# gjgjh/PTZ-Calib

Measured on AMD Instinct MI355X. Metric: LM iterations/sec (PTZ-IBA global BA, 200-view synthetic PTZ rig), higher is better.
Workload: dtype f64

## Files before the change

### __graft_entry__.py

```python
from __future__ import annotations

import importlib.util
import os
import subprocess
import sys

ROOT = os.path.dirname(os.path.abspath(__file__))
PKG_DIR = os.path.join(ROOT, "ptz-calib_amd")


def load_package():
    if "ptz_calib_amd" in sys.modules:
        return sys.modules["ptz_calib_amd"]
    spec = importlib.util.spec_from_file_location("ptz_calib_amd", os.path.join(PKG_DIR, "__init__.py"),
                                                  submodule_search_locations=[PKG_DIR])
    mod = importlib.util.module_from_spec(spec)
    sys.modules["ptz_calib_amd"] = mod
    spec.loader.exec_module(mod)
    return mod


def load_oracle():
    odir = os.path.join(ROOT, "oracle")
    if odir not in sys.path:
        sys.path.insert(0, odir)
    import oracle_py
    return oracle_py


def build() -> None:
    env = dict(os.environ)
    subprocess.check_call(["make", "-C", os.path.join(PKG_DIR, "csrc"), "-j4"], env=env)
    host = os.path.join(PKG_DIR, "host")
    if os.path.exists(os.path.join(host, "Makefile")):
        subprocess.check_call(["make", "-C", host], env=env)
    subprocess.check_call(["make", "-C", os.path.join(ROOT, "oracle")], env=env)
    harness = os.path.join(ROOT, "tests", "cpu_harness")
    for name in ("factor_harness", "homography_harness", "krt_cov_harness", "ba_cov_harness", "ba_cov_georef_harness", "pass_shape_harness",
                 "xcd_map_harness", "ba_trim_harness", "krt_trim_harness", "desc_match_harness", "desc_guided_harness", "reloc_assemble_harness",
                 "desc_shortlist_harness"):
        subprocess.check_call(["g++", "-O2", "-ffp-contract=off", "-shared", "-fPIC", "-o",
                               os.path.join(harness, "lib%s.so" % name), os.path.join(harness, name + ".cc")])
    pkg = load_package()
    pkg.api.lib()
    for name in pkg.api.EXPORTS:
        getattr(pkg.api.lib(), name)


def smoke() -> None:
    import numpy as np
    import torch

    assert torch.cuda.is_available(), "smoke() needs cuda:0"
    pkg = load_package()
    orc = load_oracle()
# ... 68 lines not shown
```

### include/ptz_calib_amd.h

```cpp
#ifndef PTZ_CALIB_AMD_H
#define PTZ_CALIB_AMD_H

#include <stdint.h>

#ifdef __cplusplus
extern "C" {
#endif

#define PTZ_CAM_DIM 15

#define PTZ_OK 0
#define PTZ_EINVAL (-1)
#define PTZ_ENODEVICE (-2)
#define PTZ_ENOMEM (-3)
#define PTZ_EUNSUPPORTED (-4)
#define PTZ_ELIMIT (-5)
#define PTZ_ENOOBS (-6)

#define PTZ_BA_PTZRay 0
#define PTZ_BA_PTZRayDist 1
#define PTZ_BA_PTZRayFxfyDist 2
#define PTZ_BA_PTZRayDistDisp 3
#define PTZ_KRT_F 0
#define PTZ_KRT_FDist 1
// ... 93 lines not shown
                       int32_t device_id, ptz_rig** out);
void ptz_rig_destroy(ptz_rig* rig);
typedef struct ptz_rig_view {
  const ptz_rig* rig;
  int32_t n_cam;
  const int32_t* cam_image;
} ptz_rig_view;
int32_t ptz_ba_batch_create_views(int32_t n, const ptz_rig_view* views, int32_t factor_type, const ptz_lm_options* opt,
                                  ptz_ba_batch** out);
int32_t ptz_ba_batch_set_state_pix2ray(ptz_ba_batch* b, const double* cam, const double* rkinv);
int32_t ptz_debug_batch_structure_hash(ptz_ba_batch* b, uint64_t* hash);
int32_t ptz_debug_batch_initial_rays(ptz_ba_batch* b, double* ray);

int32_t ptz_chol_solve_batch(int32_t count, int32_t n, const double* A, const double* rhs, double* x, int32_t* fail,
                             int32_t device_id, double* device_ms);

int32_t ptz_mfma_f64_peak(int32_t device_id, double* tflops);
int32_t ptz_ba_plan_tile_order(int32_t nt, int32_t first_dense, const uint8_t* mask, int32_t* perm, int32_t* lanes,
                               int32_t* sched, int32_t* n_steps);

int32_t ptz_hbm_bandwidth(int32_t device_id, double* read_gbps, double* copy_gbps);

int32_t ptz_krt_solve_batch(int32_t n_query, const int64_t* match_ptr, const float* uv_ref, const float* uv_cur,
                            const double* cam_ref, double* cam_cur, int32_t factor_type, double max_reproj_error,
                            const ptz_lm_options* opt, ptz_lm_summary* summaries, int32_t* accepted,
                            double* device_ms);

int32_t ptz_krt_solve_batch_2d3d(int32_t n_query, const int64_t* match_ptr, const float* uv_ref, const float* uv_cur,
                                 const int64_t* point_ptr, const float* pts2d, const double* pts3d, const double* cam_ref,
                                 double* cam_cur, int32_t factor_type, double max_reproj_error, const ptz_lm_options* opt,
// ... 282 lines not shown
```

### ptz-calib_amd/api.py

```python
from __future__ import annotations

import ctypes as C
import os

import numpy as np

_HERE = os.path.dirname(os.path.abspath(__file__))
LIB_PATH = os.environ.get("PTZCALIB_LIB", os.path.join(_HERE, "libptzcalib_hip.so"))

CONVERGENCE, NO_CONVERGENCE, FAILURE = 0, 1, 2
BA_PTZRay, BA_PTZRayDist, BA_PTZRayFxfyDist, BA_PTZRayDistDisp = 0, 1, 2, 3
KRT_F, KRT_FDist, KRT_Fxfy, KRT_FxfyDist = 0, 1, 2, 3
COV_OK, COV_DOF, COV_SINGULAR, COV_SKIPPED = 0, 1, 2, 3
PROF_SLOTS = 16
_ERR = {-1: "PTZ_EINVAL", -2: "PTZ_ENODEVICE", -3: "PTZ_ENOMEM", -4: "PTZ_EUNSUPPORTED", -5: "PTZ_ELIMIT", -6: "PTZ_ENOOBS"}

EXPORTS = ["ptz_lm_options_default", "ptz_version", "ptz_device_count", "ptz_ba_batch_create", "ptz_ba_batch_destroy",
           "ptz_ba_batch_set_state", "ptz_ba_batch_solve", "ptz_ba_batch_get_state", "ptz_ba_batch_last_solve_ms",
           "ptz_ba_batch_set_profiling", "ptz_ba_batch_get_profile", "ptz_ba_solve", "ptz_ba_cam_block_dim",
           "ptz_ba_batch_linearize", "ptz_ba_batch_pix2ray", "ptz_ba_batch_cam_block_dim", "ptz_chol_solve_batch", "ptz_krt_solve_batch",
           "ptz_krt_solve_batch_2d3d", "ptz_krt_solve_batch_device", "ptz_trim_cache", "ptz_mfma_f64_peak", "ptz_ba_solve_sharded",
           "ptz_krt_solve_batch_sharded", "ptz_hbm_bandwidth", "ptz_ba_batch_set_disp", "ptz_ba_batch_get_disp", "ptz_ba_solve_disp",
           "ptz_ba_plan_tile_order", "ptz_rig_create", "ptz_rig_destroy", "ptz_ba_batch_create_views", "ptz_ba_batch_set_state_pix2ray",
           "ptz_debug_batch_structure_hash", "ptz_debug_batch_initial_rays", "ptz_krt_table_create", "ptz_krt_table_destroy",
           "ptz_krt_solve_attempts", "ptz_homography_ransac_batch", "ptz_debug_homography_bounds", "ptz_match_gate_create",
           "ptz_match_gate_destroy", "ptz_match_gate_run_device", "ptz_match_gate_run", "ptz_krt_solve_batch_gated", "ptz_debug_match_gate_table",
           "ptz_krt_free_dim", "ptz_krt_covariance_batch", "ptz_krt_covariance_batch_device", "ptz_ba_cov_dim",
           "ptz_ba_batch_covariance", "ptz_ba_covariance", "ptz_ba_geo_cov_dim", "ptz_ba_batch_covariance_georef",
           "ptz_ba_covariance_georef", "ptz_ba_batch_residuals", "ptz_ba_batch_trim_select", "ptz_ba_problem_trim",
           "ptz_trim_options_default", "ptz_ba_solve_trimmed_batch", "ptz_ba_solve_trimmed", "ptz_krt_residuals_batch",
           "ptz_krt_residuals_batch_device", "ptz_krt_trim_options_default", "ptz_krt_trim_workspace_bytes", "ptz_krt_solve_batch_trimmed",
           "ptz_krt_solve_batch_trimmed_device", "ptz_desc_options_default", "ptz_desc_set_create", "ptz_desc_set_destroy",
           "ptz_desc_match_pairs", "ptz_desc_matches_n_matches", "ptz_desc_matches_n_pairs", "ptz_desc_matches_device_ms",
           "ptz_desc_matches_n_chunks", "ptz_desc_matches_download", "ptz_desc_matches_device_ptrs", "ptz_desc_matches_destroy",
           "ptz_debug_desc_dist2", "ptz_desc_match_pairs_guided", "ptz_desc_match_pairs_guided_device", "ptz_reloc_ref_rotations",
           "ptz_reloc_assemble_workspace_bytes", "ptz_reloc_assemble_device", "ptz_reloc_assemble", "ptz_reloc_options_default",
           "ptz_relocalizer_create", "ptz_relocalizer_destroy", "ptz_relocalizer_run", "ptz_relocalizer_n_matches", "ptz_relocalizer_matches", "ptz_relocalizer_table",
           "ptz_shortlist_options_default", "ptz_desc_shortlist", "ptz_desc_shortlist_workspace_bytes", "ptz_desc_shortlist_device",
           "ptz_relocalizer_run_shortlisted", "ptz_relocalizer_pairs"]


class PtzError(RuntimeError):
    def __init__(self, code, where):
        super().__init__(f"{where}: {_ERR.get(code, code)}")
        self.code = code


class LmOptions(C.Structure):
    _fields_ = [("max_num_iterations", C.c_int32), ("device_id", C.c_int32),
                ("max_num_consecutive_invalid_steps", C.c_int32), ("jacobi_scaling", C.c_int32),
                ("initial_trust_region_radius", C.c_double), ("max_trust_region_radius", C.c_double),
                ("min_trust_region_radius", C.c_double), ("min_relative_decrease", C.c_double),
                ("min_lm_diagonal", C.c_double), ("max_lm_diagonal", C.c_double), ("function_tolerance", C.c_double),
                ("gradient_tolerance", C.c_double), ("parameter_tolerance", C.c_double),
# ... 551 lines not shown
    if rc < 0:
        raise PtzError(rc, "ptz_ba_plan_tile_order")
    plan_tile_order.last_schedule = sched[:int(n_steps[0])]
    return bool(rc), perm, (int(lanes[0]), int(lanes[1]))


def chol_solve_batch(A, rhs, device_id=0):
    A = np.ascontiguousarray(A, dtype=np.float64)
    rhs = np.ascontiguousarray(rhs, dtype=np.float64)
    count, n = A.shape[0], A.shape[1]
    x = np.zeros((count, n))
    fail = np.zeros(count, dtype=np.int32)
    ms = C.c_double()
    _check(lib().ptz_chol_solve_batch(count, n, _p(A), _p(rhs), _p(x), _p(fail), device_id, C.byref(ms)), "ptz_chol_solve_batch")
    return x, fail, ms.value


def find_homographies(match_ptr, src_uv, dst_uv, ransac_thresh=4.0, device_id=0, mask=True):
    ptr = np.ascontiguousarray(match_ptr, dtype=np.int64)
    src = np.ascontiguousarray(src_uv, dtype=np.float32)
    dst = np.ascontiguousarray(dst_uv, dtype=np.float32)
    n = ptr.shape[0] - 1
    H = np.zeros((max(n, 0), 3, 3))
    found = np.zeros(max(n, 0), dtype=np.int32)
    m = np.zeros(int(ptr[-1]) if n > 0 else 0, dtype=np.uint8) if mask else None
    ms = C.c_double()
    _check(lib().ptz_homography_ransac_batch(n, _p(ptr), _p(src), _p(dst), C.c_double(ransac_thresh), device_id, _p(H), _p(found),
                                             _p(m), C.byref(ms)), "ptz_homography_ransac_batch")
    return H, found, m, ms.value

# ... 751 lines not shown
```

### ptz-calib_amd/csrc/ptz_ba.hip

```cpp
#include <algorithm>
#include <cmath>
#include <chrono>
#include <cstdlib>
#include <cstring>
#include <mutex>
#include <thread>
#include <vector>

#include "ptz_common.h"
#include "ptz_pool.h"
#include "ptz_factor.h"
#include "ptz_pass_shape.h"

#include "ptz_ba_kernels.h"
#include "ptz_view_kernels.h"
#include "ptz_ba_cov.h"
#include "ptz_ba_cov_georef.h"
#include "ptz_ba_resid.h"
#include <rocprim/rocprim.hpp>

namespace ptz {

enum ProfSlot { P_LIN = 0, P_LMCTL, P_RAYPREP, P_CLEAR, P_SCHUR, P_RHS, P_CHOL_PANEL, P_CHOL_SYRK, P_CHOL_BACK,
                P_BACKSUB, P_EVAL, P_SYNC, P_NSLOT };
static const char* kSlotNames[PTZ_PROF_SLOTS] = {"linearize", "lm_control", "ray_prep", "clear", "schur", "rhs",
                                                 "chol_panel", "chol_syrk", "chol_backsolve", "backsub", "eval",
                                                 "host_sync", "", "", "", ""};
// ... 347 lines not shown
    const int lo = (int)((int64_t)B * g / G), hi = (int)((int64_t)B * (g + 1) / G);
    b->group_first.push_back(lo);
    b->group_count.push_back(hi - lo);
    Dev d = b->d;
    const size_t np = d.chol.np, nt = np / CHOL_NB;
    d.n_scene = hi - lo;
    d.scene += lo; d.lm += lo; d.active += lo; d.ray_fail += lo; d.tail_cnt += 2 * (size_t)lo;
    d.yc += (size_t)lo * np;
    d.chol.count = hi - lo;
    d.chol.A += (size_t)lo * np * np;
    if (d.chol.Linv) d.chol.Linv += (size_t)lo * nt * CHOL_NB * CHOL_NB;
    d.chol.Ldiag += (size_t)lo * nt * CHOL_NB * CHOL_NB;
    d.chol.Dinv += (size_t)lo * nt * 4 * 16 * 16;
    d.chol.n += lo; d.chol.fail += lo; d.chol.active = d.active;
    if (d.chol.tmask) d.chol.tmask += (size_t)lo * nt * nt;
    if (d.chol.sched) d.chol.sched += (size_t)lo * nt * CHOL_STEP_COLS;
    if (d.tperm) { d.tperm += (size_t)lo * nt; d.chol.xperm = d.tperm; }
    d.grp_ctl = b->d_ctl + 4 * g;
    d.host_ctl = b->h_ctl_dev + 4 * g;
    d.act = b->d_act + lo;
    d.use_act = 0;
    if (d.chol.L) d.chol.L = b->d.chol.L + (size_t)g * std::min(b->n_scene, CHOL_CHAIN_SLOTS) * np * np;
    if (d.chol.chain_ctl) d.chol.chain_ctl = b->d.chol.chain_ctl + (size_t)g * chol_chain_ctl_ints((int)np);
    if (d.chol.bs_items) { d.chol.bs_items += (size_t)lo * 4 * chol_backsolve_max_groups((int)np); d.chol.bs_groups += lo; }
    b->dg.push_back(d);
  }
  if ((int)b->pass_graph.size() != G || (G > 0 && b->pass_graph[0].size() != b->shapes.size())) {
    for (auto& v : b->pass_graph) for (auto ge : v) if (ge) (void)hipGraphExecDestroy(ge);
    b->pass_graph.assign(G, std::vector<hipGraphExec_t>(b->shapes.size(), nullptr));
  }
// ... 1358 lines not shown
  TRY(b->alloc(&d.partial, (size_t)b->total_chunk * 4));
  TRY(b->alloc(&d.partial_lin, 2 * d.plin_stride));
  d.ray_block = b->ray_block;
  TRY(b->alloc(&d.camstep, (size_t)b->total_cam * 2));
  TRY(b->alloc(&d.cam_gmax, (size_t)2 * b->total_cam));
  TRY(b->alloc(&d.tail_cnt, (size_t)2 * n));
  TRY(b->alloc(&d.lm, (size_t)n));
  TRY(b->alloc(&d.active, (size_t)n));
  TRY(b->alloc(&d.ray_fail, (size_t)n));
  d.chol.count = n;
  d.chol.np = chol_padded_order(b->max_n);
  StagedUpload up2;
  std::vector<int> hn(n);
  for (int i = 0; i < n; ++i) hn[i] = b->scenes[i].n;
  up2.add(hn, &d.chol.n);
  std::vector<unsigned char> hm;
  std::vector<int> h_tperm, h_sched, h_groups;
  std::vector<BsItem> h_items;
  TRY(b->alloc(&d.chol.A, (size_t)n * d.chol.np * d.chol.np));
  {
    const int groups = std::max(1, std::min(b->n_group_hint(n), n));
    const size_t slots = (size_t)std::min(n, CHOL_CHAIN_SLOTS) * groups;
    TRY(b->alloc(&d.chol.L, slots * d.chol.np * d.chol.np));
    if (hipMemsetAsync(d.chol.L, 0, sizeof(double) * slots * d.chol.np * d.chol.np, b->io) != hipSuccess) { ptz_ba_batch_destroy(b); return PTZ_ENODEVICE; }
    TRY(b->alloc(&b->d_act, (size_t)n));
    const size_t ctl_ints = chol_chain_ctl_ints(d.chol.np) * groups;
    TRY(b->alloc(&d.chol.chain_ctl, ctl_ints));
    if (hipMemsetAsync(d.chol.chain_ctl, 0, sizeof(int) * ctl_ints, b->io) != hipSuccess) { ptz_ba_batch_destroy(b); return PTZ_ENODEVICE; }
  }
  TRY(b->alloc(&d.chol.Ldiag, (size_t)n * (d.chol.np / CHOL_NB) * CHOL_NB * CHOL_NB));
  TRY(b->alloc(&d.chol.Dinv, (size_t)n * (d.chol.np / CHOL_NB) * 4 * 16 * 16));
  TRY(b->alloc(&d.chol.Linv, (size_t)n * (d.chol.np / CHOL_NB) * CHOL_NB * CHOL_NB));
  TRY(b->alloc(&d.chol.fail, (size_t)n));
  d.chol.active = d.active;
  TRY(b->alloc(&d.yc, (size_t)n * d.chol.np));
  tc2 = now_ms();
  if (!getenv("PTZ_BA_DENSE_CHOL")) {
    const int nt = d.chol.np / CHOL_NB;
    bool dissect = true;
    bool nested = true;
    if (const char* e = getenv("PTZ_BA_ORDER")) { dissect = strcmp(e, "natural") != 0; nested = strcmp(e, "flat") != 0; }
    hm.assign((size_t)n * nt * nt, 0);
    h_tperm.resize((size_t)n * nt); h_sched.assign((size_t)n * nt * CHOL_STEP_COLS, -1);
    int max_steps = 0;
    bool any_plan = false;
    std::vector<unsigned char> m0((size_t)nt * nt);
    for (int i = 0; i < n; ++i) {
      const SceneDev& sd = b->scenes[i];
      std::fill(m0.begin(), m0.end(), 0);
      auto tile_lo = [&](int cam) { return (cam * NC) / CHOL_NB; };
      auto tile_hi = [&](int cam) { return (cam * NC + NC - 1) / CHOL_NB; };
      if (vm) memcpy(m0.data(), h_adj.data() + (size_t)i * nt * nt, (size_t)nt * nt);
      for (int c = 0; !vm && c < sd.n_cam; ++c)
        for (int a = tile_lo(c); a <= tile_hi(c); ++a)
          for (int e = tile_lo(c); e <= a; ++e) m0[a * nt + e] = 1;
      for (int p = 0; !vm && p < sd.n_pair; ++p) {
        const int ci = h_pci[sd.pair_off + p], cj = h_pcj[sd.pair_off + p];
        for (int a = tile_lo(ci); a <= tile_hi(ci); ++a)
          for (int e = tile_lo(cj); e <= tile_hi(cj); ++e) {
            if (a >= e) m0[a * nt + e] = 1; else m0[e * nt + a] = 1;
          }
// ... 18 lines not shown
      if (!planned) for (int t = 0; t < nt; ++t) perm[t] = t;
      if (planned) any_plan = true;
      unsigned char* m = hm.data() + (size_t)i * nt * nt;
      for (int a = 0; a < nt; ++a)
        for (int e = 0; e <= a; ++e) {
          if (!m0[a * nt + e]) continue;
          const int pa = perm[a], pe = perm[e];
          m[std::max(pa, pe) * nt + std::min(pa, pe)] = 1;
        }
      for (int k = 0; k < nt; ++k)
        for (int x = k + 1; x < nt; ++x) {
          if (!m[x * nt + k]) continue;
          for (int y = k + 1; y <= x; ++y)
            if (m[y * nt + k]) m[x * nt + y] = 1;
        }
      int steps = 0;
      if (planned) steps = level_schedule(nt, m, sched);
      else for (int t = 0; t < nt; ++t, ++steps) sched[CHOL_STEP_COLS * steps] = t;
      max_steps = std::max(max_steps, steps);
      if ((int)b->sched_kmin.size() < steps) b->sched_kmin.resize(steps, nt);
      for (int st = 0; st < steps; ++st) b->sched_kmin[st] = std::min(b->sched_kmin[st], sched[CHOL_STEP_COLS * st]);
      if (dbg_t && i == 0) fprintf(stderr, "[ptz_ba_create] scene 0: %d tiles, elimination %s: lanes %d + %d, %d steps\n", nt, planned ? "dissected" : "natural", lane_a, lane_b, steps);
    }
    up2.add(hm, &d.chol.tmask);
    if (any_plan) {
      up2.add(h_tperm, &d.tperm);
      up2.add(h_sched, &d.chol.sched);
      d.chol.n_steps = max_steps;
      d.chol.sched_kmin = b->sched_kmin.data();
    }
    {
      const int mg = chol_backsolve_max_groups(d.chol.np);
      const char* e = getenv("PTZ_BA_BACKSOLVE_HOST_LIST");
      if ((!e || atoi(e) != 0) && mg <= 1024 && sizeof(double) * ((size_t)d.chol.np + 1024) + sizeof(BsItem) * 4 * (size_t)mg <= 150 * 1024) {
        h_items.resize((size_t)n * 4 * mg);
        h_groups.resize(n);
        const char* es = getenv("PTZ_BA_BACKSOLVE_SPLIT");
        const bool want_split = any_plan && n <= 8 && nt <= 64 && !(es && atoi(es) == 0);
        for (int i = 0; i < n; ++i) {
// ... 876 lines not shown
```

### ptz-calib_amd/csrc/ptz_chol.hip

```cpp
#include <algorithm>
#include <atomic>
#include <cstdlib>
#include <type_traits>

#include "ptz_common.h"

namespace ptz {

namespace {

constexpr int NB = CHOL_NB;
constexpr int LD = NB + 2;

typedef double d4 __attribute__((ext_vector_type(4)));

__device__ __forceinline__ double ld_sc1(const double* p) { return __hip_atomic_load(p, __ATOMIC_RELAXED, __HIP_MEMORY_SCOPE_AGENT); }
__device__ __forceinline__ void st_sc1(double* p, double v) { __hip_atomic_store(p, v, __ATOMIC_RELAXED, __HIP_MEMORY_SCOPE_AGENT); }
typedef double d2n __attribute__((ext_vector_type(2)));
__device__ __forceinline__ void st_sc1_2(double* p, double2 v)
{
  const d2n x = {v.x, v.y};
  asm volatile("global_store_dwordx4 %0, %1, off sc1\n\ts_nop 1" : : "v"(p), "v"(x) : "memory");
}
__device__ __forceinline__ void drain_stores() { asm volatile("s_waitcnt vmcnt(0)" ::: "memory"); }
// ... 533 lines not shown
    const double* Lg = cb.Ldiag + ((size_t)sys * nt + k) * (NB * NB);
    for (int idx = threadIdx.x; idx < NBLK * DB * DB; idx += 256) {
      const int blk = idx >> 8, r = (idx >> 4) & 15, c = idx & 15;
      const int bc = blk < 1 ? 1 : (blk < 3 ? 2 : 3), bq = blk - bc * (bc - 1) / 2;
      Lb[blk * DB * LDD + r * LDD + c] = Lg[(size_t)(DB * bc + r) * NB + DB * bq + c];
    }
  }
  {
    const double* Dg = Dinv + ((size_t)sys * nt + k) * 4 * (DB * DB);
    for (int idx = threadIdx.x; idx < 4 * DB * DB; idx += 256) {
      const int b = idx >> 8, r = (idx >> 4) & 15, c = idx & 15;
      Di[b * DB * LDD + r * LDD + c] = Dg[idx];
    }
  }
  double* T = A + (size_t)(ti * NB + 16 * w) * np + k * NB;
  d4 acc[4];
#pragma unroll
  for (int c = 0; c < 4; ++c)
#pragma unroll
    for (int i = 0; i < 4; ++i) acc[c][i] = T[(size_t)(fq + 4 * i) * np + 16 * c + fr];
  __syncthreads();
  double* xs = Xs[w];
#pragma unroll
  for (int c = 0; c < 4; ++c) {
    const int slot_c = c < 3 ? c : 0;
#pragma unroll
    for (int q = 0; q < c; ++q)
#pragma unroll
      for (int ks = 0; ks < 4; ++ks) {
        const double av = -xs[fr * LDX + 16 * q + 4 * ks + fq];
        const double bv = Lb[(c * (c - 1) / 2 + q) * DB * LDD + fr * LDD + 4 * ks + fq];
        acc[c] = __builtin_amdgcn_mfma_f64_16x16x4f64(av, bv, acc[c], 0, 0, 0);
      }
    if (c == 3) __builtin_amdgcn_s_waitcnt(0xc07f);
#pragma unroll
    for (int i = 0; i < 4; ++i) xs[(fq + 4 * i) * LDX + 16 * slot_c + fr] = acc[c][i];
// ... 716 lines not shown
  __syncthreads();
  const int ticket = wg[0], gen = wg[1];
  chain_tile(cb, smem, wg, klist, ticket, gen);
  if (threadIdx.x == 0) {
    const int d = atomicAdd(&ctl[1], 1);
    if (d == total - 1) {
      __hip_atomic_store(&ctl[0], 0, __ATOMIC_RELAXED, __HIP_MEMORY_SCOPE_AGENT);
      __hip_atomic_store(&ctl[1], 0, __ATOMIC_RELAXED, __HIP_MEMORY_SCOPE_AGENT);
      __hip_atomic_store(&ctl[2], gen, __ATOMIC_RELAXED, __HIP_MEMORY_SCOPE_AGENT);
    }
  }
}

constexpr int KH = 32, LDH = KH + 2;
typedef double d8 __attribute__((ext_vector_type(8)));
__device__ __forceinline__ d8 half_fetch(const double* __restrict__ g, int ld)
{
  d8 r;
#pragma unroll
  for (int p = 0; p < (NB * KH / 2) / 256; ++p) {
    const int idx = p * 256 + threadIdx.x;
    const int row = idx >> 4, c2 = (idx & 15) * 2;
    const double2 v = *reinterpret_cast<const double2*>(g + (size_t)row * ld + c2);
    r[2 * p] = v.x; r[2 * p + 1] = v.y;
  }
  return r;
}
__global__ __launch_bounds__(256, 3) void chol_update_col_h_kernel(CholBatch cb, int j, int fuse_diag)
{
  int bx, slot;
  if (!xcd_remap(bx, slot, chol_live_rows(cb))) return;
  const int sys = chol_system_of(cb, slot);
  if (sys < 0 || (cb.active && !cb.active[sys])) return;
  const int np = cb.np, nt = np / NB;
  const int n = cb.n[sys];
  const int ti = j + bx;
  if (ti >= nt || ti * NB > n || j * NB > n) return;
  const unsigned char* tm = cb.tmask ? cb.tmask + (size_t)sys * nt * nt : nullptr;
  if (tm && !tm[ti * nt + j]) return;
  double* A = cb.A + (size_t)sys * np * np;
  __shared__ __attribute__((aligned(16))) double Ls[2 * NB * LDH];
  static_assert(2 * NB * LDH >= NB * LD, "the diagonal tile is factored in the operand buffers");
  double* As = Ls;
  double* Bs = Ls + NB * LDH;
  const int lane = threadIdx.x & 63, w = threadIdx.x >> 6;
  const int fr = lane & 15, fq = lane >> 4;
  double* C = A + (size_t)(ti * NB + 16 * w) * np + j * NB;
  d4 acc[4];
#pragma unroll
  for (int c = 0; c < 4; ++c)
#pragma unroll
    for (int i = 0; i < 4; ++i) acc[c][i] = C[(size_t)(fq + 4 * i) * np + 16 * c + fr];
  const double* ap = As + (16 * w + fr) * LDH + fq;
  const double* bp = Bs + fr * LDH + fq;
  __shared__ short klist[1024];
  __shared__ int kcount;
  if (threadIdx.x < 64) {
    const int nq = cb.sched ? CHOL_STEP_COLS * cb.n_steps : j;
    const int* sq = cb.sched ? cb.sched + (size_t)sys * nt * CHOL_STEP_COLS : nullptr;
    int cnt = 0;
    for (int q0 = 0; q0 < nq; q0 += 64) {
      const int qq = q0 + (int)threadIdx.x;
      const int kc = qq < nq ? (sq ? sq[qq] : qq) : -1;
      const bool in = kc >= 0 && kc < j;
      const bool ok = in && (!tm || (tm[ti * nt + (in ? kc : 0)] && tm[j * nt + (in ? kc : 0)]));
      const unsigned long long m = __ballot(ok);
      const int pos = cnt + __popcll(m & ((1ull << threadIdx.x) - 1ull));
      if (ok && pos < 1024) klist[pos] = (short)kc;
      cnt += __popcll(m);
    }
    if (threadIdx.x == 0) kcount = min(cnt, 1024);
  }
  __syncthreads();
  const int Q = kcount;
  auto col_of = [&](int q) { return (int)klist[q]; };
  auto next_q = [&](int q) { return q; };
  int q = 0;
  const bool any = q < Q;
  int k = any ? col_of(q) : 0;
  auto kq = [&](int qq) { return any ? col_of(qq < Q ? qq : Q - 1) : 0; };
  auto fetch_a = [&](int u) { return half_fetch(A + (size_t)(ti * NB) * np + kq(u >> 1) * NB + KH * (u & 1), np); };
  auto fetch_b = [&](int u) { return half_fetch(A + (size_t)(j * NB) * np + kq(u >> 1) * NB + KH * (u & 1), np); };
  d8 ra = fetch_a(0), rb = fetch_b(0), ra1 = fetch_a(1), rb1 = fetch_b(1);
  (void)k; (void)next_q;
  auto step = [&](d8& xa, d8& xb, int uf) {
    __syncthreads();
#pragma unroll
    for (int p = 0; p < (NB * KH / 2) / 256; ++p) {
      const int idx = p * 256 + threadIdx.x;
      const int row = idx >> 4, c2 = (idx & 15) * 2;
      *reinterpret_cast<double2*>(As + row * LDH + c2) = make_double2(-xa[2 * p], -xa[2 * p + 1]);
      *reinterpret_cast<double2*>(Bs + row * LDH + c2) = make_double2(xb[2 * p], xb[2 * p + 1]);
    }
    __syncthreads();
    xa = fetch_a(uf);
    xb = fetch_b(uf);
#pragma unroll
    for (int kk = 0; kk < KH / 4; ++kk) {
      const double av = ap[4 * kk];
#pragma unroll
      for (int c = 0; c < 4; ++c) acc[c] = __builtin_amdgcn_mfma_f64_16x16x4f64(av, bp[(16 * c) * LDH + 4 * kk], acc[c], 0, 0, 0);
    }
  };
  for (int u = 0; u < 2 * Q; u += 2) {
    step(ra, rb, u + 2);
    step(ra1, rb1, u + 3);
  }
  if (fuse_diag && ti == j) {
    __shared__ __attribute__((aligned(16))) double Dv[4][DB * LDD];
    __syncthreads();
#pragma unroll
    for (int c = 0; c < 4; ++c)
#pragma unroll
      for (int i = 0; i < 4; ++i) As[(16 * w + fq + 4 * i) * LD + 16 * c + fr] = acc[c][i];
    __syncthreads();
    diag_factor_tile(Ls, Dv, cb, sys, j, n);
    return;
  }
  if (!any) return;
#pragma unroll
  for (int c = 0; c < 4; ++c)
#pragma unroll
    for (int i = 0; i < 4; ++i) C[(size_t)(fq + 4 * i) * np + 16 * c + fr] = acc[c][i];
}

__global__ __launch_bounds__(256) void chol_tile_inverse_kernel(CholBatch cb)
{
  const int slot = blockIdx.y, k = blockIdx.x, sys = chol_system_of(cb, slot);
  if (sys < 0 || (cb.active && !cb.active[sys])) return;
  const int nt = cb.np / NB;
  if (k * NB > cb.n[sys]) return;
  __shared__ __attribute__((aligned(16))) double Lk[NB * LD];
  __shared__ __attribute__((aligned(16))) double Di[4 * DB * LDD];
  tile_g2s<256, false>(cb.Ldiag + ((size_t)sys * nt + k) * (NB * NB), NB, Lk);
// ... 325 lines not shown
void chol_factor_solve(const CholBatch& cb, double* x, hipStream_t stream)
{
  const int nt = cb.np / NB;
  if (cb.L) {
    if (chol_chain_enabled(cb)) chol_chain_launch(cb, stream);
    else {
      chol_diag_launch(cb, -1, stream);
      for (int st = 0; st + 1 < chol_step_count(cb); ++st) chol_col_step_launch(cb, st, stream);
    }
    chol_backsolve_launch(cb, x, stream);
    return;
  }
  for (int k = 0; k < nt; ++k) {
    chol_panel_launch(cb, k, stream, k > 0);
    chol_syrk_launch(cb, k, stream, 0, true);
  }
  chol_tile_inverse_launch(cb, stream);
  chol_backsolve_launch(cb, x, stream);
}

}

namespace ptz {
namespace {
__global__ __launch_bounds__(256) void mfma_f64_peak_kernel(double* out, int iters)
{
  d4 acc[8];
#pragma unroll
  for (int k = 0; k < 8; ++k) acc[k] = d4{0.0, 0.0, 0.0, 0.0};
  double a = 1.0 + 1e-9 * threadIdx.x, bq = 1.0 - 1e-9 * threadIdx.x;
// ... 88 lines not shown
    if (rep > 0 && ms < best_r) best_r = ms;
    PTZ_HIP_TRY(hipEventRecord(e0, nullptr));
    hipLaunchKernelGGL(hbm_copy_kernel, dim3(blocks), dim3(256), 0, nullptr, a, bq, n);
    PTZ_HIP_TRY(hipEventRecord(e1, nullptr));
    PTZ_HIP_TRY(hipEventSynchronize(e1));
    (void)hipEventElapsedTime(&ms, e0, e1);
    if (rep > 0 && ms < best_c) best_c = ms;
  }
  PTZ_HIP_TRY(hipGetLastError());
  *read_gbps = (double)bytes / (best_r * 1e-3) / 1e9;
  *copy_gbps = 2.0 * (double)bytes / (best_c * 1e-3) / 1e9;
  (void)hipEventDestroy(e0); (void)hipEventDestroy(e1); (void)hipFree(a); (void)hipFree(bq); (void)hipFree(d_out);
  return PTZ_OK;
}

extern "C" int32_t ptz_chol_solve_batch(int32_t count, int32_t n, const double* A, const double* rhs, double* x,
                                        int32_t* fail, int32_t device_id, double* device_ms)
{
  using namespace ptz;
  if (count <= 0 || n <= 0 || !A || !rhs || !x) return PTZ_EINVAL;
  int ndev = 0;
  if (hipGetDeviceCount(&ndev) != hipSuccess || ndev <= device_id) return PTZ_ENODEVICE;
  PTZ_DEVICE_GUARD(device_id);
  CholBatch cb;
  cb.count = count;
  cb.np = chol_padded_order(n);
  const int np = cb.np, nt = np / CHOL_NB;
  double *dA = nullptr, *dL = nullptr, *dx = nullptr, *dD = nullptr;
  int *dn = nullptr, *dfail = nullptr;
  PTZ_HIP_TRY(hipMalloc(&dA, sizeof(double) * (size_t)count * np * np));
  PTZ_HIP_TRY(hipMalloc(&dL, sizeof(double) * (size_t)count * nt * CHOL_NB * CHOL_NB));
  PTZ_HIP_TRY(hipMalloc(&dx, sizeof(double) * (size_t)count * np));
  PTZ_HIP_TRY(hipMalloc(&dD, sizeof(double) * (size_t)count * nt * 4 * 16 * 16));
  PTZ_HIP_TRY(hipMalloc(&dn, sizeof(int) * count));
  PTZ_HIP_TRY(hipMalloc(&dfail, sizeof(int) * count));
  cb.A = dA; cb.Ldiag = dL; cb.Dinv = dD; cb.n = dn; cb.fail = dfail;
  double *dL2 = nullptr, *dLi = nullptr;
  int* dctl = nullptr;
  if (count < 8) {
    PTZ_HIP_TRY(hipMalloc(&dL2, sizeof(double) * (size_t)count * np * np));
    PTZ_HIP_TRY(hipMemset(dL2, 0, sizeof(double) * (size_t)count * np * np));
    cb.L = dL2;
    PTZ_HIP_TRY(hipMalloc(&dctl, sizeof(int) * chol_chain_ctl_ints(np)));
    PTZ_HIP_TRY(hipMemset(dctl, 0, sizeof(int) * chol_chain_ctl_ints(np)));
    cb.chain_ctl = dctl;
  }
  PTZ_HIP_TRY(hipMalloc(&dLi, sizeof(double) * (size_t)count * nt * CHOL_NB * CHOL_NB));
  cb.Linv = dLi;
  {
    int* hn = new int[count];
    for (int i = 0; i < count; ++i) hn[i] = n;
    PTZ_HIP_TRY(hipMemcpy(dn, hn, sizeof(int) * count, hipMemcpyHostToDevice));
    delete[] hn;
  }
  hipStream_t stream;
  PTZ_HIP_TRY(hipStreamCreate(&stream));
  hipEvent_t e0, e1;
  PTZ_HIP_TRY(hipEventCreate(&e0));
  PTZ_HIP_TRY(hipEventCreate(&e1));
  chol_clear(cb, stream);
  for (int s = 0; s < count; ++s) {
    PTZ_HIP_TRY(hipMemcpy2DAsync(dA + (size_t)s * np * np, sizeof(double) * np, A + (size_t)s * n * n, sizeof(double) * n,
                                 sizeof(double) * n, n, hipMemcpyHostToDevice, stream));
    PTZ_HIP_TRY(hipMemcpyAsync(dA + (size_t)s * np * np + (size_t)n * np, rhs + (size_t)s * n, sizeof(double) * n,
                               hipMemcpyHostToDevice, stream));
  }
  PTZ_HIP_TRY(hipEventRecord(e0, stream));
  chol_factor_solve(cb, dx, stream);
  PTZ_HIP_TRY(hipEventRecord(e1, stream));
  PTZ_HIP_TRY(hipStreamSynchronize(stream));
  float ms = 0;
  (void)hipEventElapsedTime(&ms, e0, e1);
  if (device_ms) *device_ms = ms;
  for (int s = 0; s < count; ++s)
    PTZ_HIP_TRY(hipMemcpy(x + (size_t)s * n, dx + (size_t)s * np, sizeof(double) * n, hipMemcpyDeviceToHost));
  bool lost = false;
  {
    int* hf = new int[count];
    PTZ_HIP_TRY(hipMemcpy(hf, dfail, sizeof(int) * count, hipMemcpyDeviceToHost));
    for (int s = 0; s < count; ++s) { lost |= (hf[s] & 2) != 0; if (fail) fail[s] = hf[s] & 1; }
    delete[] hf;
  }
  (void)hipEventDestroy(e0); (void)hipEventDestroy(e1); (void)hipStreamDestroy(stream);
  (void)hipFree(dA); (void)hipFree(dL); (void)hipFree(dD); (void)hipFree(dx); (void)hipFree(dn); (void)hipFree(dfail);
  if (dL2) (void)hipFree(dL2);
  if (dLi) (void)hipFree(dLi);
  if (dctl) (void)hipFree(dctl);
  return lost ? PTZ_ENODEVICE : PTZ_OK;
}
```

### ptz-calib_amd/csrc/ptz_common.h

```cpp
#pragma once

#include <hip/hip_runtime.h>
#include <stdint.h>
#include <stdio.h>
#include <string.h>

#include <chrono>
#include <thread>
#include <tuple>
#include <utility>

#include "../../include/ptz_calib_amd.h"
#include "ptz_xcd_map.h"

namespace ptz {

#define PTZ_HIP_TRY(expr)                                                                      \
  do {                                                                                         \
    hipError_t _e = (expr);                                                                    \
    if (_e != hipSuccess) {                                                                    \
      fprintf(stderr, "[ptzcalib] HIP error %s at %s:%d: %s\n", hipGetErrorName(_e), __FILE__, \
              __LINE__, #expr);                                                                \
      return (_e == hipErrorOutOfMemory) ? PTZ_ENOMEM : PTZ_ENODEVICE;                         \
    }                                                                                          \
// ... 173 lines not shown
      double t = scratch[k];
      for (int i = 1; i < nw; ++i) t = fmax(t, scratch[4 * i + k]);
      v[k] = t;
    }
    else {
      double t = 0;
      for (int i = 0; i < nw; ++i) t += scratch[4 * i + k];
      v[k] = t;
    }
  }
}

constexpr int CHOL_NB = 64;
constexpr double CHOL_BIG = 1e300;
constexpr int CHOL_STEP_COLS = 4;
struct CholBatch {
  int count = 0;
  int np = 0;
  double* A = nullptr;
  double* L = nullptr;
  double* Linv = nullptr;
  const int* act = nullptr;
  const int* act_n = nullptr;
  int xcd_live = 1;
  double* Ldiag = nullptr;
  double* Dinv = nullptr;
  const int* n = nullptr;
  int* fail = nullptr;
  const int* active = nullptr;
  const unsigned char* tmask = nullptr;
  const int* sched = nullptr;
  int n_steps = 0;
  const int* sched_kmin = nullptr;
  int* chain_ctl = nullptr;
  int chain_spin_limit = 0;
  const struct BsItem* bs_items = nullptr;
  const int* bs_groups = nullptr;
  int bs_split = 0;
  const int* xperm = nullptr;
};
struct BsItem { long long off; int ld, in_off, out_off, kind; };
inline int chol_backsolve_max_groups(int np)
{
  const int nt = np / CHOL_NB;
  int g = nt;
// ... 82 lines not shown
}
constexpr int CHOL_CHAIN_SLOTS = 32;
inline size_t chol_chain_ctl_ints(int np) { const size_t nt = (size_t)np / CHOL_NB; return 4 + (size_t)CHOL_CHAIN_SLOTS * (4 * nt + nt * nt); }
bool chol_chain_fits(int count, int np);
__device__ __forceinline__ int chol_system_of(const CholBatch& cb, int slot)
{
  if (!cb.act) return slot;
  return slot < *cb.act_n ? cb.act[slot] : -1;
}
__device__ __forceinline__ unsigned chol_live_rows(const CholBatch& cb)
{
  return (cb.act && cb.xcd_live) ? (unsigned)max(*cb.act_n, 0) : gridDim.y;
}
inline int chol_padded_order(int n_max) { return ((n_max + 1 + CHOL_NB - 1) / CHOL_NB) * CHOL_NB; }
void chol_factor_solve(const CholBatch& cb, double* x, hipStream_t stream);
void chol_panel_launch(const CholBatch& cb, int k, hipStream_t stream, bool diag_done = false);
void chol_syrk_launch(const CholBatch& cb, int k, hipStream_t stream, int mode, bool fuse_diag = false);
void chol_backsolve_launch(const CholBatch& cb, double* x, hipStream_t stream);
void chol_tile_inverse_launch(const CholBatch& cb, hipStream_t stream);
void chol_diag_launch(const CholBatch& cb, int k, hipStream_t stream);
bool chol_chain_enabled(const CholBatch& cb);
void chol_chain_launch(const CholBatch& cb, hipStream_t stream);
inline int chol_step_count(const CholBatch& cb) { return cb.sched ? cb.n_steps : cb.np / CHOL_NB; }
void chol_col_step_launch(const CholBatch& cb, int k, hipStream_t stream);
void chol_update_col_launch(const CholBatch& cb, int j, hipStream_t stream, bool fuse_diag = false);
void chol_clear(const CholBatch& cb, hipStream_t stream);
#ifdef PTZ_CHOL_TIMELINE
void chol_chain_timeline_print(int nt);
#endif

// ... 2 lines not shown
```

Before: 67880.

## Skip zero 16-row strips in blocked Cholesky loads using a strip sparsity mask

Adds a per-tile strip mask that records which 16-row strips of each 64x64 tile can be nonzero, built from the camera-pair structure on the host. The update and panel kernels then read from a shared zero line instead of global memory for empty strips, and skip writeback of dead strips. The aim is to cut memory traffic in the batched Cholesky used by the BA solve. It also adds a left-looking structured solve entry point and a test harness. The cost is extra mask lookups, scalar branching, and fallback logic when the strip mask disagrees with the tile mask.

```diff
diff --git a/__graft_entry__.py b/__graft_entry__.py
--- a/__graft_entry__.py
+++ b/__graft_entry__.py
@@ -38,7 +38,7 @@
     harness = os.path.join(ROOT, "tests", "cpu_harness")
     for name in ("factor_harness", "homography_harness", "krt_cov_harness", "ba_cov_harness", "ba_cov_georef_harness", "pass_shape_harness",
                  "xcd_map_harness", "ba_trim_harness", "krt_trim_harness", "desc_match_harness", "desc_guided_harness", "reloc_assemble_harness",
-                 "desc_shortlist_harness"):
+                 "desc_shortlist_harness", "chol_strips_harness"):
         subprocess.check_call(["g++", "-O2", "-ffp-contract=off", "-shared", "-fPIC", "-o",
                                os.path.join(harness, "lib%s.so" % name), os.path.join(harness, name + ".cc")])
     pkg = load_package()
diff --git a/include/ptz_calib_amd.h b/include/ptz_calib_amd.h
--- a/include/ptz_calib_amd.h
+++ b/include/ptz_calib_amd.h
@@ -131,6 +131,9 @@
 
 int32_t ptz_chol_solve_batch(int32_t count, int32_t n, const double* A, const double* rhs, double* x, int32_t* fail,
                              int32_t device_id, double* device_ms);
+int32_t ptz_chol_solve_batch_structured(int32_t count, int32_t n, const double* A, const double* rhs, const uint8_t* tmask,
+                                        const uint8_t* smask, double* x, double* L, int32_t* fail, int32_t device_id);
+int32_t ptz_chol_left_looking_min_count(int32_t n);
 
 int32_t ptz_mfma_f64_peak(int32_t device_id, double* tflops);
 int32_t ptz_ba_plan_tile_order(int32_t nt, int32_t first_dense, const uint8_t* mask, int32_t* perm, int32_t* lanes,
diff --git a/ptz-calib_amd/api.py b/ptz-calib_amd/api.py
--- a/ptz-calib_amd/api.py
+++ b/ptz-calib_amd/api.py
@@ -37,7 +37,8 @@
            "ptz_reloc_assemble_workspace_bytes", "ptz_reloc_assemble_device", "ptz_reloc_assemble", "ptz_reloc_options_default",
            "ptz_relocalizer_create", "ptz_relocalizer_destroy", "ptz_relocalizer_run", "ptz_relocalizer_n_matches", "ptz_relocalizer_matches", "ptz_relocalizer_table",
            "ptz_shortlist_options_default", "ptz_desc_shortlist", "ptz_desc_shortlist_workspace_bytes", "ptz_desc_shortlist_device",
-           "ptz_relocalizer_run_shortlisted", "ptz_relocalizer_pairs"]
+           "ptz_relocalizer_run_shortlisted", "ptz_relocalizer_pairs", "ptz_chol_solve_batch_structured",
+           "ptz_chol_left_looking_min_count"]
 
 
 class PtzError(RuntimeError):
@@ -619,6 +620,26 @@
     ms = C.c_double()
     _check(lib().ptz_chol_solve_batch(count, n, _p(A), _p(rhs), _p(x), _p(fail), device_id, C.byref(ms)), "ptz_chol_solve_batch")
     return x, fail, ms.value
+
+
+def chol_left_looking_min_count(n):
+    return int(lib().ptz_chol_left_looking_min_count(int(n)))
+
+
+def chol_solve_batch_structured(A, rhs, tmask, smask=None, device_id=0):
+    A = np.ascontiguousarray(A, dtype=np.float64)
+    rhs = np.ascontiguousarray(rhs, dtype=np.float64)
+    count, n = A.shape[0], A.shape[1]
+    npad = (n + 1 + 63) // 64 * 64
+    tmask = np.ascontiguousarray(tmask, dtype=np.uint8)
+    smask = None if smask is None else np.ascontiguousarray(smask, dtype=np.uint8)
+    assert tmask.shape == (npad // 64, npad // 64) and (smask is None or smask.shape == tmask.shape)
+    x = np.zeros((count, n))
+    L = np.zeros((count, npad, npad))
+    fail = np.zeros(count, dtype=np.int32)
+    _check(lib().ptz_chol_solve_batch_structured(count, n, _p(A), _p(rhs), _p(tmask), _p(smask), _p(x), _p(L), _p(fail), device_id),
+           "ptz_chol_solve_batch_structured")
+    return x, L, fail
 
 
 def find_homographies(match_ptr, src_uv, dst_uv, ransac_thresh=4.0, device_id=0, mask=True):
diff --git a/ptz-calib_amd/csrc/ptz_ba.hip b/ptz-calib_amd/csrc/ptz_ba.hip
--- a/ptz-calib_amd/csrc/ptz_ba.hip
+++ b/ptz-calib_amd/csrc/ptz_ba.hip
@@ -11,6 +11,7 @@
 #include "ptz_pool.h"
 #include "ptz_factor.h"
 #include "ptz_pass_shape.h"
+#include "ptz_chol_strips.h"
 
 #include "ptz_ba_kernels.h"
 #include "ptz_view_kernels.h"
@@ -388,6 +389,7 @@
     d.chol.Dinv += (size_t)lo * nt * 4 * 16 * 16;
     d.chol.n += lo; d.chol.fail += lo; d.chol.active = d.active;
     if (d.chol.tmask) d.chol.tmask += (size_t)lo * nt * nt;
+    if (d.chol.smask) d.chol.smask += (size_t)lo * nt * nt;
     if (d.chol.sched) d.chol.sched += (size_t)lo * nt * CHOL_STEP_COLS;
     if (d.tperm) { d.tperm += (size_t)lo * nt; d.chol.xperm = d.tperm; }
     d.grp_ctl = b->d_ctl + 4 * g;
@@ -1776,7 +1778,7 @@
   std::vector<int> hn(n);
   for (int i = 0; i < n; ++i) hn[i] = b->scenes[i].n;
   up2.add(hn, &d.chol.n);
-  std::vector<unsigned char> hm;
+  std::vector<unsigned char> hm, hs;
   std::vector<int> h_tperm, h_sched, h_groups;
   std::vector<BsItem> h_items;
   TRY(b->alloc(&d.chol.A, (size_t)n * d.chol.np * d.chol.np));
@@ -1807,6 +1809,9 @@
     int max_steps = 0;
     bool any_plan = false;
     std::vector<unsigned char> m0((size_t)nt * nt);
+    bool strips = !vm && !any_shared;
+    if (const char* e = getenv("PTZ_BA_CHOL_STRIPS")) strips = strips && atoi(e) != 0;
+    if (strips) hs.assign((size_t)n * nt * nt, 0);
     for (int i = 0; i < n; ++i) {
       const SceneDev& sd = b->scenes[i];
       std::fill(m0.begin(), m0.end(), 0);
@@ -1855,6 +1860,14 @@
           for (int y = k + 1; y <= x; ++y)
             if (m[y * nt + k]) m[x * nt + y] = 1;
         }
+      if (strips) {
+        StripWriters w;
+        w.n = sd.n; w.n_cam = sd.n_cam; w.nc = NC; w.dense_row = sd.n_cam * NC;
+        w.n_pair = sd.n_pair; w.pair_ci = h_pci.data() + sd.pair_off; w.pair_cj = h_pcj.data() + sd.pair_off;
+        unsigned char* sm = hs.data() + (size_t)i * nt * nt;
+        chol_strip_mask(nt, w, perm, sm);
+        if (!chol_strip_mask_matches(nt, sd.n, m, sm)) strips = false;
+      }
       int steps = 0;
       if (planned) steps = level_schedule(nt, m, sched);
       else for (int t = 0; t < nt; ++t, ++steps) sched[CHOL_STEP_COLS * steps] = t;
@@ -1864,6 +1877,13 @@
       if (dbg_t && i == 0) fprintf(stderr, "[ptz_ba_create] scene 0: %d tiles, elimination %s: lanes %d + %d, %d steps\n", nt, planned ? "dissected" : "natural", lane_a, lane_b, steps);
     }
     up2.add(hm, &d.chol.tmask);
+    if (strips) {
+      double* zl = nullptr;
+      TRY(b->alloc(&zl, chol_zline_bytes(d.chol.np) / sizeof(double)));
+      if (hipMemsetAsync(zl, 0, chol_zline_bytes(d.chol.np), b->io) != hipSuccess) { ptz_ba_batch_destroy(b); return PTZ_ENODEVICE; }
+      d.chol.zline = zl;
+      up2.add(hs, &d.chol.smask);
+    }
     if (any_plan) {
       up2.add(h_tperm, &d.tperm);
       up2.add(h_sched, &d.chol.sched);
diff --git a/ptz-calib_amd/csrc/ptz_chol.hip b/ptz-calib_amd/csrc/ptz_chol.hip
--- a/ptz-calib_amd/csrc/ptz_chol.hip
+++ b/ptz-calib_amd/csrc/ptz_chol.hip
@@ -2,6 +2,7 @@
 #include <atomic>
 #include <cstdlib>
 #include <type_traits>
+#include <vector>
 
 #include "ptz_common.h"
 
@@ -571,12 +572,15 @@
     }
   }
   double* T = A + (size_t)(ti * NB + 16 * w) * np + k * NB;
+  const bool live = !cb.smask || ((cb.smask[((size_t)sys * nt + ti) * nt + k] >> __builtin_amdgcn_readfirstlane(w)) & 1);
+  const double* Tl = live ? T : cb.zline;
   d4 acc[4];
 #pragma unroll
   for (int c = 0; c < 4; ++c)
 #pragma unroll
-    for (int i = 0; i < 4; ++i) acc[c][i] = T[(size_t)(fq + 4 * i) * np + 16 * c + fr];
+    for (int i = 0; i < 4; ++i) acc[c][i] = Tl[live ? (size_t)(fq + 4 * i) * np + 16 * c + fr : 0];
   __syncthreads();
+  if (!live) return;
   double* xs = Xs[w];
 #pragma unroll
   for (int c = 0; c < 4; ++c) {
@@ -1323,14 +1327,14 @@
 
 constexpr int KH = 32, LDH = KH + 2;
 typedef double d8 __attribute__((ext_vector_type(8)));
-__device__ __forceinline__ d8 half_fetch(const double* __restrict__ g, int ld)
+__device__ __forceinline__ d8 half_fetch(const double* __restrict__ g, int ld, unsigned strips, const double* __restrict__ zl)
 {
   d8 r;
+  const unsigned off = (threadIdx.x >> 4) * (unsigned)ld + (threadIdx.x & 15) * 2;
 #pragma unroll
   for (int p = 0; p < (NB * KH / 2) / 256; ++p) {
-    const int idx = p * 256 + threadIdx.x;
-    const int row = idx >> 4, c2 = (idx & 15) * 2;
-    const double2 v = *reinterpret_cast<const double2*>(g + (size_t)row * ld + c2);
+    const double* base = ((strips >> p) & 1u) ? g + (size_t)(16 * p) * ld : zl;
+    const double2 v = *reinterpret_cast<const double2*>(base + off);
     r[2 * p] = v.x; r[2 * p + 1] = v.y;
   }
   return r;
@@ -1355,14 +1359,11 @@
   const int lane = threadIdx.x & 63, w = threadIdx.x >> 6;
   const int fr = lane & 15, fq = lane >> 4;
   double* C = A + (size_t)(ti * NB + 16 * w) * np + j * NB;
-  d4 acc[4];
-#pragma unroll
-  for (int c = 0; c < 4; ++c)
-#pragma unroll
-    for (int i = 0; i < 4; ++i) acc[c][i] = C[(size_t)(fq + 4 * i) * np + 16 * c + fr];
+  const unsigned char* sm = cb.smask ? cb.smask + (size_t)sys * nt * nt : nullptr;
+  const double* zl = cb.zline;
   const double* ap = As + (16 * w + fr) * LDH + fq;
   const double* bp = Bs + fr * LDH + fq;
-  __shared__ short klist[1024];
+  __shared__ int kent[1024];
   __shared__ int kcount;
   if (threadIdx.x < 64) {
     const int nq = cb.sched ? CHOL_STEP_COLS * cb.n_steps : j;
@@ -1373,26 +1374,33 @@
       const int kc = qq < nq ? (sq ? sq[qq] : qq) : -1;
       const bool in = kc >= 0 && kc < j;
       const bool ok = in && (!tm || (tm[ti * nt + (in ? kc : 0)] && tm[j * nt + (in ? kc : 0)]));
+      const int st = sm ? (sm[ti * nt + (in ? kc : 0)] & 15) | ((sm[j * nt + (in ? kc : 0)] & 15) << 4) : 0xFF;
       const unsigned long long m = __ballot(ok);
       const int pos = cnt + __popcll(m & ((1ull << threadIdx.x) - 1ull));
-      if (ok && pos < 1024) klist[pos] = (short)kc;
+      if (ok && pos < 1024) kent[pos] = kc | (st << 16);
       cnt += __popcll(m);
     }
-    if (threadIdx.x == 0) kcount = min(cnt, 1024);
+    if (threadIdx.x == 0) { kcount = min(cnt, 1024); if (cnt == 0) kent[0] = 0; }
   }
   __syncthreads();
   const int Q = kcount;
-  auto col_of = [&](int q) { return (int)klist[q]; };
-  auto next_q = [&](int q) { return q; };
-  int q = 0;
-  const bool any = q < Q;
-  int k = any ? col_of(q) : 0;
-  auto kq = [&](int qq) { return any ? col_of(qq < Q ? qq : Q - 1) : 0; };
-  auto fetch_a = [&](int u) { return half_fetch(A + (size_t)(ti * NB) * np + kq(u >> 1) * NB + KH * (u & 1), np); };
-  auto fetch_b = [&](int u) { return half_fetch(A + (size_t)(j * NB) * np + kq(u >> 1) * NB + KH * (u & 1), np); };
-  d8 ra = fetch_a(0), rb = fetch_b(0), ra1 = fetch_a(1), rb1 = fetch_b(1);
-  (void)k; (void)next_q;
-  auto step = [&](d8& xa, d8& xb, int uf) {
+  const bool any = Q > 0;
+  const bool c_live = !sm || ((sm[ti * nt + j] >> __builtin_amdgcn_readfirstlane(w)) & 1);
+  const bool c_read = c_live && (any || (fuse_diag && ti == j) || !zl);
+  const double* Cl = c_read ? C : zl;
+  d4 acc[4];
+#pragma unroll
+  for (int c = 0; c < 4; ++c)
+#pragma unroll
+    for (int i = 0; i < 4; ++i) acc[c][i] = Cl[c_read ? (size_t)(fq + 4 * i) * np + 16 * c + fr : 0];
+  const unsigned past = zl ? 0u : 0xFFu;
+  auto entry = [&](int qq) { return __builtin_amdgcn_readfirstlane(kent[any ? min(qq, Q - 1) : 0]); };
+  auto fetch_a = [&](int e, unsigned st, int h) { return half_fetch(A + (size_t)(ti * NB) * np + (e & 0xFFFF) * NB + KH * h, np, st & 15u, zl); };
+  auto fetch_b = [&](int e, unsigned st, int h) { return half_fetch(A + (size_t)(j * NB) * np + (e & 0xFFFF) * NB + KH * h, np, st >> 4, zl); };
+  const int e0 = entry(0);
+  const unsigned s0 = any ? (unsigned)e0 >> 16 : past;
+  d8 ra = fetch_a(e0, s0, 0), rb = fetch_b(e0, s0, 0), ra1 = fetch_a(e0, s0, 1), rb1 = fetch_b(e0, s0, 1);
+  auto step = [&](d8& xa, d8& xb, int e, unsigned st, int h) {
     __syncthreads();
 #pragma unroll
     for (int p = 0; p < (NB * KH / 2) / 256; ++p) {
@@ -1402,8 +1410,9 @@
       *reinterpret_cast<double2*>(Bs + row * LDH + c2) = make_double2(xb[2 * p], xb[2 * p + 1]);
     }
     __syncthreads();
-    xa = fetch_a(uf);
-    xb = fetch_b(uf);
+    asm volatile("" : "+s"(e), "+s"(st));
+    xa = fetch_a(e, st, h);
+    xb = fetch_b(e, st, h);
 #pragma unroll
     for (int kk = 0; kk < KH / 4; ++kk) {
       const double av = ap[4 * kk];
@@ -1411,9 +1420,11 @@
       for (int c = 0; c < 4; ++c) acc[c] = __builtin_amdgcn_mfma_f64_16x16x4f64(av, bp[(16 * c) * LDH + 4 * kk], acc[c], 0, 0, 0);
     }
   };
-  for (int u = 0; u < 2 * Q; u += 2) {
-    step(ra, rb, u + 2);
-    step(ra1, rb1, u + 3);
+  for (int q = 0; q < Q; ++q) {
+    const int e = entry(q + 1);
+    const unsigned st = q + 1 < Q ? (unsigned)e >> 16 : past;
+    step(ra, rb, e, st, 0);
+    step(ra1, rb1, e, st, 1);
   }
   if (fuse_diag && ti == j) {
     __shared__ __attribute__((aligned(16))) double Dv[4][DB * LDD];
@@ -1426,7 +1437,7 @@
     diag_factor_tile(Ls, Dv, cb, sys, j, n);
     return;
   }
-  if (!any) return;
+  if (!any || !c_live) return;
 #pragma unroll
   for (int c = 0; c < 4; ++c)
 #pragma unroll
@@ -1782,6 +1793,17 @@
   for (int k = 0; k < nt; ++k) {
     chol_panel_launch(cb, k, stream, k > 0);
     chol_syrk_launch(cb, k, stream, 0, true);
+  }
+  chol_tile_inverse_launch(cb, stream);
+  chol_backsolve_launch(cb, x, stream);
+}
+
+void chol_factor_solve_left(const CholBatch& cb, double* x, hipStream_t stream)
+{
+  const int nt = cb.np / NB;
+  for (int k = 0; k < nt; ++k) {
+    if (k > 0) chol_update_col_launch(cb, k, stream, true);
+    chol_panel_launch(cb, k, stream, k > 0);
   }
   chol_tile_inverse_launch(cb, stream);
   chol_backsolve_launch(cb, x, stream);
@@ -1900,8 +1922,8 @@
   return PTZ_OK;
 }
 
-extern "C" int32_t ptz_chol_solve_batch(int32_t count, int32_t n, const double* A, const double* rhs, double* x,
-                                        int32_t* fail, int32_t device_id, double* device_ms)
+static int32_t chol_solve_batch_impl(int32_t count, int32_t n, const double* A, const double* rhs, double* x, int32_t* fail, int32_t device_id,
+                                     double* device_ms, const uint8_t* tmask, const uint8_t* smask, double* Lout)
 {
   using namespace ptz;
   if (count <= 0 || n <= 0 || !A || !rhs || !x) return PTZ_EINVAL;
@@ -1923,7 +1945,29 @@
   cb.A = dA; cb.Ldiag = dL; cb.Dinv = dD; cb.n = dn; cb.fail = dfail;
   double *dL2 = nullptr, *dLi = nullptr;
   int* dctl = nullptr;
-  if (count < 8) {
+  const bool few = tmask ? (count <= 8 || chol_chain_fits(count, np)) : count < 8;
+  unsigned char *dtm = nullptr, *dsm = nullptr;
+  double* dzl = nullptr;
+  if (tmask) {
+    if (count > CHOL_CHAIN_SLOTS && few) return PTZ_EINVAL;
+    const char* e = getenv("PTZ_BA_CHOL_STRIPS");
+    const bool strips = smask && !(e && atoi(e) == 0);
+    std::vector<unsigned char> rep((size_t)count * nt * nt);
+    PTZ_HIP_TRY(hipMalloc(&dtm, rep.size()));
+    for (int s = 0; s < count; ++s) std::copy(tmask, tmask + nt * nt, rep.begin() + (size_t)s * nt * nt);
+    PTZ_HIP_TRY(hipMemcpy(dtm, rep.data(), rep.size(), hipMemcpyHostToDevice));
+    cb.tmask = dtm;
+    if (strips) {
+      PTZ_HIP_TRY(hipMalloc(&dsm, rep.size()));
+      for (int s = 0; s < count; ++s) std::copy(smask, smask + nt * nt, rep.begin() + (size_t)s * nt * nt);
+      PTZ_HIP_TRY(hipMemcpy(dsm, rep.data(), rep.size(), hipMemcpyHostToDevice));
+      PTZ_HIP_TRY(hipMalloc(&dzl, chol_zline_bytes(np)));
+      PTZ_HIP_TRY(hipMemset(dzl, 0, chol_zline_bytes(np)));
+      cb.smask = dsm; cb.zline = dzl;
+    }
+    PTZ_HIP_TRY(hipMemset(dA, 0, sizeof(double) * (size_t)count * np * np));
+  }
+  if (few) {
     PTZ_HIP_TRY(hipMalloc(&dL2, sizeof(double) * (size_t)count * np * np));
     PTZ_HIP_TRY(hipMemset(dL2, 0, sizeof(double) * (size_t)count * np * np));
     cb.L = dL2;
@@ -1952,7 +1996,8 @@
                                hipMemcpyHostToDevice, stream));
   }
   PTZ_HIP_TRY(hipEventRecord(e0, stream));
-  chol_factor_solve(cb, dx, stream);
+  if (tmask && !few) chol_factor_solve_left(cb, dx, stream);
+  else chol_factor_solve(cb, dx, stream);
   PTZ_HIP_TRY(hipEventRecord(e1, stream));
   PTZ_HIP_TRY(hipStreamSynchronize(stream));
   float ms = 0;
@@ -1967,10 +2012,44 @@
     for (int s = 0; s < count; ++s) { lost |= (hf[s] & 2) != 0; if (fail) fail[s] = hf[s] & 1; }
     delete[] hf;
   }
+  if (Lout) {
+    PTZ_HIP_TRY(hipMemcpy(Lout, cb.L ? dL2 : dA, sizeof(double) * (size_t)count * np * np, hipMemcpyDeviceToHost));
+    std::vector<double> ld((size_t)count * nt * CHOL_NB * CHOL_NB);
+    PTZ_HIP_TRY(hipMemcpy(ld.data(), dL, sizeof(double) * ld.size(), hipMemcpyDeviceToHost));
+    for (int s = 0; s < count; ++s)
+      for (int t = 0; t < nt; ++t)
+        for (int r = 0; r < CHOL_NB; ++r)
+          std::copy(ld.begin() + ((size_t)(s * nt + t) * CHOL_NB + r) * CHOL_NB, ld.begin() + ((size_t)(s * nt + t) * CHOL_NB + r + 1) * CHOL_NB,
+                    Lout + (size_t)s * np * np + (size_t)(t * CHOL_NB + r) * np + t * CHOL_NB);
+  }
   (void)hipEventDestroy(e0); (void)hipEventDestroy(e1); (void)hipStreamDestroy(stream);
   (void)hipFree(dA); (void)hipFree(dL); (void)hipFree(dD); (void)hipFree(dx); (void)hipFree(dn); (void)hipFree(dfail);
   if (dL2) (void)hipFree(dL2);
   if (dLi) (void)hipFree(dLi);
   if (dctl) (void)hipFree(dctl);
+  if (dtm) (void)hipFree(dtm);
+  if (dsm) (void)hipFree(dsm);
+  if (dzl) (void)hipFree(dzl);
   return lost ? PTZ_ENODEVICE : PTZ_OK;
 }
+
+extern "C" int32_t ptz_chol_solve_batch(int32_t count, int32_t n, const double* A, const double* rhs, double* x,
+                                        int32_t* fail, int32_t device_id, double* device_ms)
+{
+  return chol_solve_batch_impl(count, n, A, rhs, x, fail, device_id, device_ms, nullptr, nullptr, nullptr);
+}
+
+extern "C" int32_t ptz_chol_solve_batch_structured(int32_t count, int32_t n, const double* A, const double* rhs, const uint8_t* tmask,
+                                                   const uint8_t* smask, double* x, double* L, int32_t* fail, int32_t device_id)
+{
+  if (!tmask) return PTZ_EINVAL;
+  return chol_solve_batch_impl(count, n, A, rhs, x, fail, device_id, nullptr, tmask, smask, L);
+}
+
+extern "C" int32_t ptz_chol_left_looking_min_count(int32_t n)
+{
+  const int np = ptz::chol_padded_order(n);
+  int count = 9;
+  while (count < (1 << 20) && ptz::chol_chain_fits(count, np)) ++count;
+  return count;
+}
diff --git a/ptz-calib_amd/csrc/ptz_chol_strips.h b/ptz-calib_amd/csrc/ptz_chol_strips.h
--- /dev/null
+++ b/ptz-calib_amd/csrc/ptz_chol_strips.h
@@ -0,0 +1,65 @@
+#pragma once
+
+#include <algorithm>
+
+namespace ptz {
+
+constexpr int CHOL_STRIP = 16;
+constexpr int CHOL_STRIP_TILE = 64;
+constexpr int CHOL_STRIPS = CHOL_STRIP_TILE / CHOL_STRIP;
+constexpr unsigned char CHOL_STRIPS_ALL = (1u << CHOL_STRIPS) - 1u;
+static_assert(CHOL_STRIPS <= 8, "a tile's strips fit one byte");
+
+struct StripWriters {
+  int n = 0;
+  int n_cam = 0;
+  int nc = 0;
+  int n_pair = 0;
+  const int* pair_ci = nullptr;
+  const int* pair_cj = nullptr;
+  int dense_row = 0;
+  int n_rep = 0;
+  const int* rep_cam = nullptr;
+};
+
+inline void chol_strip_mask(int nt, const StripWriters& w, const int* tperm, unsigned char* sm)
+{
+  const int NB = CHOL_STRIP_TILE;
+  std::fill(sm, sm + (size_t)nt * nt, (unsigned char)0);
+  auto pos = [&](int c) { return (tperm ? tperm[c / NB] : c / NB) * NB + c % NB; };
+  auto mark = [&](int r, int c) {
+    int pr = pos(r), pc = pos(c);
+    if (pr < pc) std::swap(pr, pc);
+    sm[(size_t)(pr / NB) * nt + pc / NB] |= (unsigned char)(1u << ((pr % NB) / CHOL_STRIP));
+  };
+  auto block = [&](int ci, int cj) {
+    for (int a = 0; a < w.nc; ++a)
+      for (int e = 0; e < w.nc; ++e) mark(ci * w.nc + a, cj * w.nc + e);
+  };
+  for (int c = 0; c < w.n_cam; ++c) block(c, c);
+  for (int p = 0; p < w.n_pair; ++p) block(w.pair_ci[p], w.pair_cj[p]);
+  for (int r = w.dense_row; r <= w.n && r < nt * NB; ++r)
+    for (int c = 0; c <= r; ++c) mark(r, c);
+  for (int g = 0; g < w.n_rep; ++g)
+    for (int a = 0; a < w.nc; ++a)
+      for (int c = 0; c <= w.n && c < nt * NB; ++c) mark(w.rep_cam[g] * w.nc + a, c);
+  for (int t = 0; t < nt; ++t) sm[(size_t)t * nt + t] = CHOL_STRIPS_ALL;
+  for (int k = 0; k < nt; ++k)
+    for (int x = k + 1; x < nt; ++x) {
+      const unsigned char s = sm[(size_t)x * nt + k];
+      if (!s) continue;
+      for (int y = k + 1; y < x; ++y)
+        if (sm[(size_t)y * nt + k]) sm[(size_t)x * nt + y] |= s;
+    }
+}
+
+inline bool chol_strip_mask_matches(int nt, int n, const unsigned char* tm, const unsigned char* sm)
+{
+  const int rows = std::min(nt, n / CHOL_STRIP_TILE + 1);
+  for (int i = 0; i < rows; ++i)
+    for (int k = 0; k <= i; ++k)
+      if ((tm[(size_t)i * nt + k] != 0) != (sm[(size_t)i * nt + k] != 0)) return false;
+  return true;
+}
+
+}
diff --git a/ptz-calib_amd/csrc/ptz_common.h b/ptz-calib_amd/csrc/ptz_common.h
--- a/ptz-calib_amd/csrc/ptz_common.h
+++ b/ptz-calib_amd/csrc/ptz_common.h
@@ -211,6 +211,7 @@
 constexpr int CHOL_NB = 64;
 constexpr double CHOL_BIG = 1e300;
 constexpr int CHOL_STEP_COLS = 4;
+inline size_t chol_zline_bytes(int np) { return sizeof(double) * (15 * (size_t)np + 32); }
 struct CholBatch {
   int count = 0;
   int np = 0;
@@ -226,6 +227,8 @@
   int* fail = nullptr;
   const int* active = nullptr;
   const unsigned char* tmask = nullptr;
+  const unsigned char* smask = nullptr;
+  const double* zline = nullptr;
   const int* sched = nullptr;
   int n_steps = 0;
   const int* sched_kmin = nullptr;
@@ -338,6 +341,7 @@
 }
 inline int chol_padded_order(int n_max) { return ((n_max + 1 + CHOL_NB - 1) / CHOL_NB) * CHOL_NB; }
 void chol_factor_solve(const CholBatch& cb, double* x, hipStream_t stream);
+void chol_factor_solve_left(const CholBatch& cb, double* x, hipStream_t stream);
 void chol_panel_launch(const CholBatch& cb, int k, hipStream_t stream, bool diag_done = false);
 void chol_syrk_launch(const CholBatch& cb, int k, hipStream_t stream, int mode, bool fuse_diag = false);
 void chol_backsolve_launch(const CholBatch& cb, double* x, hipStream_t stream);
```

After: 67970 (median of 2 runs). About the same (+0.1%).
